# mlysy/rodeo

Hardware: AMD Instinct MI355X
Metric: ODE steps/sec x batch (trajectory-steps/s), FitzHugh-Nagumo q=3, 4000 steps, solve_mv (higher is better)
Workload: dtype f64

## Files before the change

### rodeo_amd/csrc/embed_sources.py

```python
#!/usr/bin/env python3
import os
import sys

HEADERS = ["rk_enums.hpp", "linalg_small.hpp", "kalman_small.hpp", "philox.hpp", "solve_args.hpp", "dual.hpp",
           "sqrt_small.hpp", "solve_small_kernels.hpp", "mfma_tile.hpp", "solve_tile3_kernels.hpp",
           "solve_tile4_kernels.hpp", "solve_tilen_kernels.hpp", "solve_sqrt_kernels.hpp", "solve_small_m_kernels.hpp",
           "solve_dense_itg_kernels.hpp", "dalton_kernels.hpp", "dalton_tile3_kernels.hpp", "rhs.hpp", "dual2.hpp",
           "daltonng_kernels.hpp", "dalton_at_kernels.hpp", "dalton_at_tile3_kernels.hpp", "evidence_kernels.hpp",
           "evidence_tile3_kernels.hpp", "dynamic_kernels.hpp"]
here = os.path.dirname(os.path.abspath(__file__))
out = sys.argv[1]
with open(out, "w") as f:
    f.write("// generated by embed_sources.py -- do not edit\n")
    f.write("static const char* const kJitHeaderNames[] = {%s};\n" % ", ".join('"%s"' % h for h in HEADERS))
    f.write("static const char* const kJitHeaderSources[] = {\n")
    for h in HEADERS:
        src = open(os.path.join(here, h)).read()
        assert ')RKSRC"' not in src
        chunks = [src[i:i + 8000] for i in range(0, len(src), 8000)]
        f.write("    " + "\n    ".join('R"RKSRC(%s)RKSRC"' % c for c in chunks) + ",\n")
    f.write("};\nstatic const int kJitNumHeaders = %d;\n" % len(HEADERS))
```

### rodeo_amd/csrc/solve_args.hpp

```cpp
#pragma once
#ifndef __HIPCC_RTC__
#include <hip/hip_runtime.h>
#endif
#include <stdint.h>

namespace rk {

struct SolveArgs {
    int B, N, D;
    double t_min, t_max;
    uint64_t seed, traj_offset;
    const double *W, *x0, *Q, *R, *theta;
    int W_b, x0_b, Q_b, R_b, theta_b;
    double *mean, *var, *mean_pred, *var_pred, *x;
};

__device__ __forceinline__ double ld(const double* p, size_t e, int batched, int B, int b) {
    return batched ? p[e * (size_t)B + b] : p[e];
}

template <int P>
__device__ __forceinline__ void load_block_consts(const SolveArgs& a, int blk, int b, double (&Q)[P][P],
                                                  double (&R)[P][P]) {
#pragma unroll
    for (int i = 0; i < P; ++i)
#pragma unroll
        for (int j = 0; j < P; ++j) {
            const size_t e = ((size_t)blk * P + i) * P + j;
            Q[i][j] = ld(a.Q, e, a.Q_b, a.B, b);
            R[i][j] = ld(a.R, e, a.R_b, a.B, b);
        }
}

}
```

### rodeo_amd/csrc/solve_tile3.hip

```cpp
#include <cstdlib>
#include "common.hpp"
#include "kalman_small.hpp"
#include "mfma_tile.hpp"
#include "philox.hpp"
#include "rhs.hpp"
#include "solve_args.hpp"
#include "solve_paths.hpp"
#include "solve_tile3_kernels.hpp"
#include "fenrir_at_args.hpp"

namespace rk {

constexpr int CHUNK = 16;
constexpr int ITEM_BYTES = 3 * 128;
constexpr int BUF_BYTES = CHUNK * 4 * ITEM_BYTES;
constexpr int ZONE_BYTES = 64 * TILE_DOUBLES * 8;

__device__ __forceinline__ int lds_byte(int s, int g, int which, int idx) {
    const int item = s * 4 + g;
    return item * ITEM_BYTES + which * 128 + (tile_slot(s, g, idx) << 3);
}

__device__ __forceinline__ void tile3_gain_producers(const SolveArgs& a, const double* __restrict__ tiles, int D, int tw, int wave,
                                                     int lane, int n_tiles, size_t tstride, int n_chunks, char* lds_raw,
                                                     char* zones) {
    constexpr int P = 3;
    const int p = wave - 1;
    const int s = lane >> 2, g = lane & 3;
    int tau = tw * 4 + g;
    if (tau >= n_tiles) tau = n_tiles - 1;
    const int b = tau / D, blk = tau - b * D;
    double Q[P][P], R[P][P];
    load_block_consts<P>(a, blk, b, Q, R);
    int woff[12];
#pragma unroll
    for (int i = 0; i < 3; ++i)
#pragma unroll
        for (int j = 0; j < 4; ++j) woff[i * 4 + j] = lds_byte(s, g, 0, i * 4 + j);
    char* const zone = zones + p * ZONE_BYTES;
    const unsigned zone_lds = __builtin_amdgcn_readfirstlane(lds_addr(zone));
    int frow[6], fcol[6];
#pragma unroll
    for (int i = 0; i < 6; ++i) { const int j = 64 * i + lane; frow[i] = j / 24; fcol[i] = (j % 24) * 16; }
    const char* const wave_tiles = (const char*)(tiles + (size_t)tw * 4 * TILE_DOUBLES);
    auto fetch = [&](int ch) {
        const int n_hi = a.N - 1 - ch * CHUNK;
#pragma unroll
        for (int i = 0; i < 6; ++i) {
            const int n = n_hi - frow[i];
            lds_dma16(wave_tiles + (size_t)(n < 1 ? 1 : n) * tstride * 8 + fcol[i], zone_lds + 1024 * i);
        }
    };
    lds_dma_wait_all();
    if (p < n_chunks) fetch(p);
    double mf[P], Sf[P][P], mp[P], Sp[P][P], A[P][P], X[P][P], rpiv[P];
    for (int t = -3; t < n_chunks; ++t) {
        const int ch1 = t + 3, ch2 = t + 2, ch3 = t + 1;
        if (ch1 % 3 == p) {
            if (ch1 < n_chunks) {
                lds_dma_wait_all();
                double buf[TILE_DOUBLES];
#pragma unroll
                for (int k = 0; k < 6; ++k) {
                    const double2 v = *(const double2*)(zone + 96 * lane + 16 * k);
                    buf[2 * k] = v.x; buf[2 * k + 1] = v.y;
                }
                lds_reads_done();
                if (ch1 + 3 < n_chunks) fetch(ch1 + 3);
#pragma unroll
                for (int i = 0; i < P; ++i) {
#pragma unroll
                    for (int j = 0; j < P; ++j) Sf[i][j] = buf[i * 4 + j];
                    mf[i] = buf[i * 4 + 3];
                }
                predict_block<P>(Q, R, mf, Sf, mp, Sp);
            }
        } else if (ch2 >= 0 && ch2 % 3 == p) {
            if (ch2 < n_chunks) {
                double T[P][P];
                mm_nt<P, P, P>(Sf, Q, T);
#pragma unroll
                for (int i = 0; i < P; ++i)
#pragma unroll
                    for (int j = 0; j < P; ++j) { A[i][j] = Sp[i][j]; X[i][j] = T[j][i]; }
                lu_factor_fwd<P, P>(A, X, rpiv);
            }
        } else if (ch3 >= 0) {
            if (ch3 < n_chunks) {
                lu_back<P, P>(A, X, rpiv);
                const int n = a.N - 1 - ch3 * CHUNK - s;
                if (n >= 1) {
                    char* o = lds_raw + (ch3 & 1) * BUF_BYTES;
#pragma unroll
                    for (int i = 0; i < P; ++i) {
#pragma unroll
                        for (int j = 0; j < P; ++j) {
                            *(double*)(o + woff[i * 4 + j]) = Sp[i][j];
                            *(double*)(o + woff[i * 4 + j] + 128) = X[i][j];
                            *(double*)(o + woff[i * 4 + j] + 256) = Sf[i][j];
                        }
                        *(double*)(o + woff[i * 4 + 3]) = mp[i];
                        *(double*)(o + woff[i * 4 + 3] + 256) = mf[i];
                    }
                }
            }
        }
        lds_barrier();   
    }
}

__global__ void __launch_bounds__(256) bwd_mv_tile3_kernel(SolveArgs a, double* __restrict__ tiles, int D) {
    __shared__ __attribute__((aligned(16))) char lds_all[2 * BUF_BYTES];
    __shared__ __attribute__((aligned(16))) char zones[3 * ZONE_BYTES];
    const int wave = threadIdx.x >> 6, lane = threadIdx.x & 63;
    const int n_tiles = a.B * D;
    const size_t tstride = (size_t)n_tiles * TILE_DOUBLES;
    const int n_chunks = (a.N - 1 + CHUNK - 1) / CHUNK;

    for (int i = threadIdx.x; i < 2 * 64 * 3 * 16; i += 256) {
        const int idx = i & 15, which = (i >> 4) % 3, item = ((i >> 4) / 3) & 63, buf = i / (64 * 3 * 16);
        const double v = (idx == 15) ? 1.0 : 0.0;
        *(double*)(lds_all + buf * BUF_BYTES + lds_byte(item >> 2, item & 3, which, idx)) = v;
    }
    __syncthreads();

    const int tw = blockIdx.x;
    char* const lds_raw = lds_all;
    double* const dump = tiles + (size_t)(a.N + 1) * tstride + (size_t)tw * 64;
    const int role = wave;

    if (role >= 1) {
        tile3_gain_producers(a, tiles, D, tw, role, lane, n_tiles, tstride, n_chunks, lds_raw, zones);
    } else {
        const TileCoord tc = tile_coord<1>(tw, lane, n_tiles);
        __builtin_amdgcn_s_setprio(3);
        const int r = tc.r, g = tc.g, c = tc.c, idx = r * 4 + c;
        const bool st = tc.valid && r < 3;
        double* base = st ? tiles + (size_t)tc.tau * TILE_DOUBLES + idx : dump + lane;
        const size_t ostride = st ? tstride : 0;
        int roff[4];
#pragma unroll
        for (int k = 0; k < 4; ++k) roff[k] = lds_byte(k, g, 0, idx) - k * 4 * ITEM_BYTES;
        double Ms = st ? base[(size_t)a.N * ostride] : ((r == 3 && c == 3) ? 1.0 : 0.0);
        const char* const wave_rows = (const char*)(tiles + (size_t)tw * 4 * TILE_DOUBLES);
        const size_t row_bytes = tstride * sizeof(double);
        const unsigned bvoff = st ? (unsigned)((g * TILE_DOUBLES + idx) * sizeof(double)) : 0x80000000u;
        const bool buffer_ok = (CHUNK - 1) * row_bytes + 384 < 0x7fffffffull;
        const int chunk_span = (int)((CHUNK - 1) * row_bytes + 384);
        lds_barrier();
        lds_barrier();
        lds_barrier();
        for (int t = 0; t < n_chunks; ++t) {
            const char* in = lds_raw + (t & 1) * BUF_BYTES;
            const int n_hi = a.N - 1 - t * CHUNK;
            const int cnt = __builtin_amdgcn_readfirstlane(n_hi >= CHUNK ? CHUNK : n_hi);
            double* o = base + (size_t)n_hi * ostride;
            {
                if (cnt == CHUNK && buffer_ok) {
                    constexpr int LOOKAHEAD = 4;
                    double Mp[CHUNK], Gt[CHUNK], Mf[CHUNK];
                    auto load = [&](int s) {
                        const char* q = in + roff[s & 3] + s * 4 * ITEM_BYTES;
                        Mp[s] = *(const double*)(q);
                        Gt[s] = *(const double*)(q + 128);
                        Mf[s] = *(const double*)(q + 256);
                    };
#pragma unroll
                    for (int s = 0; s < LOOKAHEAD; ++s) load(s);
                    const __amdgpu_buffer_rsrc_t rsrc = __builtin_amdgcn_make_buffer_rsrc(
                        (void*)(wave_rows + (size_t)(n_hi - (CHUNK - 1)) * row_bytes), 0, chunk_span, 0x00020000);
                    double Dm = Ms - Mp[0];
#pragma unroll
                    for (int s = 0; s < CHUNK; ++s) {
                        if (s + LOOKAHEAD < CHUNK) load(s + LOOKAHEAD);
                        __builtin_amdgcn_sched_barrier(0);
                        const double V1 = MF(Dm, Gt[s], 0.0);
                        Ms = MF(V1, Gt[s], Mf[s]);
                        if (s + 1 < CHUNK) Dm = Ms - Mp[s + 1];
                        u32x2 bits;
                        __builtin_memcpy(&bits, &Ms, 8);
                        __builtin_amdgcn_raw_buffer_store_b64(bits, rsrc, (int)bvoff, (int)((CHUNK - 1 - s) * row_bytes), 0);
                        __builtin_amdgcn_sched_barrier(0);
                    }
                } else {
                    for (int s = 0; s < cnt; ++s) {
                        const char* q = in + lds_byte(s, g, 0, idx);
                        const double Mp = *(const double*)(q), Gt = *(const double*)(q + 128), Mf = *(const double*)(q + 256);
                        const double V1 = MF(Ms - Mp, Gt, 0.0);
                        Ms = MF(V1, Gt, Mf);
                        o[0] = Ms;
                        o -= ostride;
                    }
                }
            }
            lds_barrier();   
        }
    }
}

struct FenrirObs {
    const double *obs, *obs_w, *obs_v;
    const int32_t* obs_ind;
    int n_obs;
    double* logdens;
};

template <bool AT, class OB>
__device__ __forceinline__ void fenrir_tile3_body(const SolveArgs& a, const double* __restrict__ tiles, int D, const OB& ob) {
    __shared__ __attribute__((aligned(16))) char lds_all[2 * BUF_BYTES];
    __shared__ __attribute__((aligned(16))) char zones[3 * ZONE_BYTES];
    const int wave = threadIdx.x >> 6, lane = threadIdx.x & 63;
    const int n_tiles = a.B * D;
    const size_t tstride = (size_t)n_tiles * TILE_DOUBLES;
    const int n_chunks = (a.N - 1 + CHUNK - 1) / CHUNK;

    for (int i = threadIdx.x; i < 2 * 64 * 3 * 16; i += 256) {
        const int idx = i & 15, which = (i >> 4) % 3, item = ((i >> 4) / 3) & 63, buf = i / (64 * 3 * 16);
        const double v = (idx == 15) ? 1.0 : 0.0;
        *(double*)(lds_all + buf * BUF_BYTES + lds_byte(item >> 2, item & 3, which, idx)) = v;
    }
    __syncthreads();

    const int tw = blockIdx.x;
    char* const lds_raw = lds_all;

    if (wave >= 1) {
        tile3_gain_producers(a, tiles, D, tw, wave, lane, n_tiles, tstride, n_chunks, lds_raw, zones);
    } else {
        __builtin_amdgcn_s_setprio(3);
        const int r = lane >> 4, g = (lane >> 2) & 3, c = lane & 3, idx = r * 4 + c;
        const int tau_raw = tw * 4 + g;
        const bool valid = tau_raw < n_tiles;
        const int tau = valid ? tau_raw : n_tiles - 1;
        const int b = tau / D, blk = tau - b * D;
        const bool in_tile = valid && r < 3;
        const double e3 = (r == 3 && c == 3) ? 1.0 : 0.0, I4 = r == c ? 1.0 : 0.0;
        const double* const my = tiles + (size_t)tau * TILE_DOUBLES + idx;
        int roff[4];
#pragma unroll
        for (int k = 0; k < 4; ++k) roff[k] = lds_byte(k, g, 0, idx) - k * 4 * ITEM_BYTES;
        double Ms = in_tile ? my[(size_t)a.N * tstride] : e3;
        double acc = 0.0;
        int i = ob.n_obs - 1;
        int next = -1;
        [[maybe_unused]] int off = 0;
        auto look = [&]() {
            if constexpr (AT) {
                next = i >= 0 ? ob.tab[4 * i] : -1;
                off = i >= 0 ? ob.tab[4 * i + 1] : 0;
            } else {
                next = i >= 0 ? ob.obs_ind[i] : -1;
            }
        };
        look();
        auto observe = [&]() {
            const double xw = valid ? (r < 3 ? ob.obs_w[((size_t)i * D + blk) * 3 + r] : -ob.obs[(size_t)i * D + blk]) : 0.0;
            const double Om = valid ? ob.obs_v[(size_t)i * D + blk] : 1.0;
            double MsT = MF(Ms, I4, 0.0);
            MsT = r == 3 ? 0.0 : MsT;
            const double WS = MF(xw, Ms, 0.0);
            const double Z = MF(MsT, xw, 0.0);
            const double w = MF(Z, xw, 0.0) + Om;
            const double z = -quad_bcast3(WS);
            if (fabs(w) > 1e-8) acc += -0.5 * (z * z / w + log(w)) - 0.5 * 1.83787706640934548356;
            const double K = Z / w;
            Ms = fma(-K, WS, Ms);
            --i;
            look();
        };
        auto step = [&](double Mp, double Gt, double Mf) {
            const double V1 = MF(Ms - Mp, Gt, 0.0);
            Ms = MF(V1, Gt, Mf);
        };
        [[maybe_unused]] auto interval = [&](int n, bool to_node) {
            if constexpr (AT) {
                const double* const my_hops = ob.hops + (size_t)tau * FENRIR_AT_TILE_REC + idx;
                const int n_rec = ob.n_pre + ob.n_post;
                auto hop = [&](int rec) {
                    const double* q = my_hops + (size_t)fenrir_at_clamp(rec, n_rec) * n_tiles * FENRIR_AT_TILE_REC;
                    step(q[0], q[16], q[32]);
                };
                hop(ob.n_pre + fenrir_at_clamp(ob.tab[4 * i + 3], ob.n_post));
                do {
                    const int pre = fenrir_at_clamp(ob.tab[4 * i + 2], ob.n_pre);
                    observe();
                    if (to_node || (off && next == n)) hop(pre);
                } while (off && next == n);
            }
        };
        if (next >= a.N && !off) observe();
        __syncthreads();
        __syncthreads();
        __syncthreads();
        for (int t = 0; t < n_chunks; ++t) {
            const char* in = lds_raw + (t & 1) * BUF_BYTES;
            const int n_hi = a.N - 1 - t * CHUNK;
            const int cnt = __builtin_amdgcn_readfirstlane(n_hi >= CHUNK ? CHUNK : n_hi);
            const bool has_obs = next > n_hi - cnt;
            if (cnt == CHUNK && !has_obs) {
                constexpr int LOOKAHEAD = 4;
                double Mp[CHUNK], Gt[CHUNK], Mf[CHUNK];
                auto load = [&](int s) {
                    const char* q = in + roff[s & 3] + s * 4 * ITEM_BYTES;
                    Mp[s] = *(const double*)(q);
                    Gt[s] = *(const double*)(q + 128);
                    Mf[s] = *(const double*)(q + 256);
                };
#pragma unroll
                for (int s = 0; s < LOOKAHEAD; ++s) load(s);
                double Dm = Ms - Mp[0];
#pragma unroll
                for (int s = 0; s < CHUNK; ++s) {
                    if (s + LOOKAHEAD < CHUNK) load(s + LOOKAHEAD);
                    __builtin_amdgcn_sched_barrier(0);
                    const double V1 = MF(Dm, Gt[s], 0.0);
                    Ms = MF(V1, Gt[s], Mf[s]);
                    if (s + 1 < CHUNK) Dm = Ms - Mp[s + 1];
                    __builtin_amdgcn_sched_barrier(0);
                }
            } else {
                for (int s = 0; s < cnt; ++s) {
                    const int n = n_hi - s;
                    bool hops = false;
                    if constexpr (AT) hops = off && next == n;
                    if (hops) {
                        interval(n, true);
                    } else {
                        const char* q = in + lds_byte(s, g, 0, idx);
                        step(*(const double*)(q), *(const double*)(q + 128), *(const double*)(q + 256));
                    }
                    if (!off && next == n) observe();
                }
            }
            __syncthreads();
        }
        if constexpr (AT)
            if (off && next == 0) interval(0, false);
        if (!off && next == 0) {
            Ms = in_tile ? my[0] : e3;
            observe();
        }
        if (valid && r == 0 && c == 0) atomicAdd(&ob.logdens[b], acc);
    }
}

__global__ void __launch_bounds__(256) fenrir_bwd_tile3_kernel(SolveArgs a, const double* __restrict__ tiles, int D, FenrirObs ob) {
    fenrir_tile3_body<false>(a, tiles, D, ob);
}

__global__ void __launch_bounds__(256) fenrir_bwd_at_tile3_kernel(SolveArgs a, const double* __restrict__ tiles, int D, FenrirAt ob) {
    fenrir_tile3_body<true>(a, tiles, D, ob);
}

constexpr int SIM_ITEM = 256;
constexpr int SIM_BUF = CHUNK * 4 * SIM_ITEM;

__device__ __forceinline__ int sim_tile_byte(int s, int g, int idx) {
    const int item = s * 4 + g;
    return item * SIM_ITEM + (tile_slot(s, g, idx) << 3);
}
__device__ __forceinline__ int sim_vec_byte(int s, int g, int which, int rr) {
    const int item = s * 4 + g;
    return item * SIM_ITEM + 128 + (vec_slot(s, g, which, rr) << 3);
}

struct SimLogpost {
    const double* obs;
    const int32_t* obs_ind;
    int n_obs;
    double noise_sd;
    const double* upars;
    int n_prior;
    double prior_sd;
    double* logpost;
};
constexpr int LP_MAX_OBS = 512, LP_MAX_VALS = 1024;

template <bool LP>
__global__ void __launch_bounds__(256, 2) bwd_sim_tile3_kernel(SolveArgs a, double* __restrict__ tiles, int D, SimLogpost lp) {
    constexpr int P = 3;
    __shared__ double lp_obs[LP ? LP_MAX_VALS : 1];
    __shared__ int lp_ind[LP ? LP_MAX_OBS : 1];
    if constexpr (LP) {
        for (int i = threadIdx.x; i < lp.n_obs * D; i += 256) lp_obs[i] = lp.obs[i];
        for (int i = threadIdx.x; i < lp.n_obs; i += 256) { const int ni = lp.obs_ind[i]; lp_ind[i] = ni < 0 ? 0 : (ni > a.N ? a.N : ni); }
    }
    __shared__ __attribute__((aligned(16))) char lds_all[2 * SIM_BUF];
    __shared__ __attribute__((aligned(16))) char zones[3 * ZONE_BYTES];
    constexpr int QR_STRIDE = 2 * 9 + 2;
    __shared__ __attribute__((aligned(16))) double qr[4 * QR_STRIDE];
    const int wave = threadIdx.x >> 6, lane = threadIdx.x & 63;
    const int n_tiles = a.B * D;
    const size_t tstride = (size_t)n_tiles * TILE_DOUBLES;
    const int n_chunks = (a.N + CHUNK - 1) / CHUNK;
    for (int i = threadIdx.x; i < 2 * SIM_BUF / 8; i += 256) ((double*)lds_all)[i] = 0.0;
    __syncthreads();
    const int tw = blockIdx.x;
    char* const lds_raw = lds_all;
    double* const dump = tiles + (size_t)(a.N + 1) * tstride + (size_t)tw * 64;

    if (wave >= 1) {
        const int p = wave - 1;
        const int s = lane >> 2, g = lane & 3;
        int tau = tw * 4 + g;
        if (tau >= n_tiles) tau = n_tiles - 1;
        const int b = tau / D, blk = tau - b * D;
        const uint32_t traj = (uint32_t)(a.traj_offset + (uint64_t)b);
        if (p == 0 && s == 0) {
            double Q0[P][P], R0[P][P];
            load_block_consts<P>(a, blk, b, Q0, R0);
#pragma unroll
            for (int i = 0; i < P; ++i)
#pragma unroll
                for (int j = 0; j < P; ++j) { qr[g * QR_STRIDE + i * P + j] = Q0[i][j]; qr[g * QR_STRIDE + 9 + i * P + j] = R0[i][j]; }
        }
        lds_barrier();
        const double* const my_qr = qr + g * QR_STRIDE;
        auto load_q = [&](double (&Qv)[P][P]) {
#pragma unroll
            for (int i = 0; i < P; ++i)
#pragma unroll
                for (int j = 0; j < P; ++j) Qv[i][j] = my_qr[i * P + j];
        };
        int woff[9], voff[3], voff1[3];
#pragma unroll
        for (int i = 0; i < 3; ++i) {
#pragma unroll
            for (int j = 0; j < 3; ++j) woff[i * 3 + j] = sim_tile_byte(s, g, i * 4 + j);
            voff[i] = sim_vec_byte(s, g, 0, i);
            voff1[i] = sim_vec_byte(s, g, 1, i);
        }
        char* const zone = zones + p * ZONE_BYTES;
        const unsigned zone_lds = __builtin_amdgcn_readfirstlane(lds_addr(zone));
        int frow[6], fcol[6];
#pragma unroll
        for (int i = 0; i < 6; ++i) { const int j = 64 * i + lane; frow[i] = j / 24; fcol[i] = (j % 24) * 16; }
        const char* const wave_tiles = (const char*)(tiles + (size_t)tw * 4 * TILE_DOUBLES);
        auto fetch = [&](int ch) {
            const int n_hi = a.N - ch * CHUNK;
#pragma unroll
            for (int i = 0; i < 6; ++i) {
                const int n = n_hi - frow[i];
                lds_dma16(wave_tiles + (size_t)(n < 1 ? 1 : n) * tstride * 8 + fcol[i], zone_lds + 1024 * i);
            }
        };
        lds_dma_wait_all();
        if (p < n_chunks) fetch(p);
        double mf[P], Sf[P][P], mp[P], Sp[P][P], T[P][P], A[P][P], X[P][P], rpiv[P], z[P];
        for (int t = -3; t < n_chunks; ++t) {
            const int ch1 = t + 3, ch2 = t + 2, ch3 = t + 1;
            if (ch1 % 3 == p) {
                if (ch1 < n_chunks) {
                    lds_dma_wait_all();
                    double buf[TILE_DOUBLES];
#pragma unroll
                    for (int k = 0; k < 6; ++k) {
                        const double2 v = *(const double2*)(zone + 96 * lane + 16 * k);
                        buf[2 * k] = v.x; buf[2 * k + 1] = v.y;
                    }
                    lds_reads_done();
                    if (ch1 + 3 < n_chunks) fetch(ch1 + 3);
#pragma unroll
                    for (int i = 0; i < P; ++i) {
#pragma unroll
                        for (int j = 0; j < P; ++j) Sf[i][j] = buf[i * 4 + j];
                        mf[i] = buf[i * 4 + 3];
                    }
                    {
                        double Q[P][P], R[P][P];
                        load_q(Q);
#pragma unroll
                        for (int i = 0; i < P; ++i)
#pragma unroll
                            for (int j = 0; j < P; ++j) R[i][j] = my_qr[9 + i * P + j];
                        predict_block<P>(Q, R, mf, Sf, mp, Sp);
                    }
                    const int n = a.N - ch1 * CHUNK - s;
#ifdef RK_T3_ABLATE_SIMZ
                    z[0] = 0.25 + 1e-3 * n; z[1] = -0.5;
#else
                    normal_pair(a.seed, traj, (uint32_t)(n < 1 ? 1 : n), (uint32_t)blk, PURPOSE_SMOOTH, 0u, z[0], z[1]);
#endif
                }
            } else if (ch2 >= 0 && ch2 % 3 == p) {
                if (ch2 < n_chunks) {
                    {
                        double Q[P][P];
                        load_q(Q);
                        mm_nt<P, P, P>(Sf, Q, T);
                    }
#pragma unroll
                    for (int i = 0; i < P; ++i)
#pragma unroll
                        for (int j = 0; j < P; ++j) { A[i][j] = Sp[i][j]; X[i][j] = T[j][i]; }
                    lu_factor_fwd<P, P>(A, X, rpiv);
                    const int n = a.N - ch2 * CHUNK - s;
                    double z3;
#ifdef RK_T3_ABLATE_SIMZ
                    z[2] = 0.125 + 1e-3 * n; z3 = 0.0;
#else
                    normal_pair(a.seed, traj, (uint32_t)(n < 1 ? 1 : n), (uint32_t)blk, PURPOSE_SMOOTH, 1u, z[2], z3);
#endif
                }
            } else if (ch3 >= 0) {
                if (ch3 < n_chunks) {
                    const int n = a.N - ch3 * CHUNK - s;
                    double GT[P][P], Ssim[P][P], L[P][P], G[P][P];
                    lu_back<P, P>(A, X, rpiv);
                    const bool term = n == a.N;
#pragma unroll
                    for (int i = 0; i < P; ++i)
#pragma unroll
                        for (int j = 0; j < P; ++j) G[i][j] = term ? 0.0 : X[j][i];
                    mm_nt<P, P, P>(G, T, GT);
#pragma unroll
                    for (int i = 0; i < P; ++i)
#pragma unroll
                        for (int j = 0; j < P; ++j) Ssim[i][j] = Sf[i][j] - GT[i][j];
#ifdef RK_T3_ABLATE_SIMPSD
#pragma unroll
                    for (int i = 0; i < P; ++i)
#pragma unroll
                        for (int j = 0; j < P; ++j) L[i][j] = Ssim[i][j];
#else
                    psd_factor<P>(Ssim, L);
#endif
                    if (n >= 1) {
                        char* o = lds_raw + (ch3 & 1) * SIM_BUF;
#pragma unroll
                        for (int i = 0; i < P; ++i) {
                            double w = mf[i];
#pragma unroll
                            for (int k = 0; k <= i; ++k) w = fma(L[i][k], z[k], w);
#pragma unroll
                            for (int j = 0; j < P; ++j) *(double*)(o + woff[i * 3 + j]) = G[j][i];
                            *(double*)(o + voff[i]) = term ? 0.0 : mp[i];
                            *(double*)(o + voff1[i]) = w;
                        }
                    }
                }
            }
            lds_barrier();
        }
    } else {
        const TileCoord tc = tile_coord<1>(tw, lane, n_tiles);
        const int r = tc.r, g = tc.g, c = tc.c, idx = r * 4 + c;
        const int b = tc.tau / D, blk = tc.tau - b * D;
        const bool st = tc.valid && r < 3 && c == 0 && a.x != nullptr;
        const size_t xstride = (size_t)D * P * a.B;
        double* bx = st ? a.x + ((size_t)blk * P + r) * a.B + b : dump + lane;
        const double LOG_SQRT_2PI = 0.91893853320467274178;
        const double lsd = LP ? log(lp.noise_sd) : 0.0;
        int io = LP ? lp.n_obs - 1 : -1;
        double acc = 0.0;
        auto next_index = [&]() { return io >= 0 ? __builtin_amdgcn_readfirstlane(lp_ind[io]) : -1; };
        auto observe = [&](double xv) {
            const double zz = (lp_obs[io * D + blk] - xv) / lp.noise_sd;
            acc += -0.5 * zz * zz - lsd - LOG_SQRT_2PI;
            --io;
        };
        const size_t sx = st ? xstride : 0;
        const bool xbuf_ok = (size_t)CHUNK * xstride * sizeof(double) < 0x7fffffffull;
        const int xvo = st && xbuf_ok ? (int)((((size_t)blk * P + r) * a.B + b) * sizeof(double)) : (int)0x80000000;
        int roff[4], rvec[4], rvec1[4];
#pragma unroll
        for (int k = 0; k < 4; ++k) {
            roff[k] = sim_tile_byte(k, g, idx) - k * 4 * SIM_ITEM;
            rvec[k] = sim_vec_byte(k, g, 0, r) - k * 4 * SIM_ITEM;
            rvec1[k] = sim_vec_byte(k, g, 1, r) - k * 4 * SIM_ITEM;
        }
        double x = 0.0;
        lds_barrier();
        int next_n = LP ? next_index() : -1;
        lds_barrier();
        lds_barrier();
        lds_barrier();
        for (int t = 0; t < n_chunks; ++t) {
            const char* in = lds_raw + (t & 1) * SIM_BUF;
            const int n_hi = a.N - t * CHUNK;
            const int cnt = __builtin_amdgcn_readfirstlane(n_hi >= CHUNK ? CHUNK : n_hi);
            double* o = bx + (size_t)n_hi * sx;
            auto step = [&](const char* q, const char* qv, const char* qw) {
                const double Gt = *(const double*)(q), mp = *(const double*)(qv), mfw = *(const double*)(qw);
                x = MF(Gt, x - mp, mfw);
                o[0] = x;
                o -= sx;
            };
            int n_cur = n_hi;
            if (cnt == CHUNK && xbuf_ok) {
                const __amdgpu_buffer_rsrc_t rsrc = __builtin_amdgcn_make_buffer_rsrc(
                    (void*)(a.x + (size_t)(n_hi - (CHUNK - 1)) * xstride), 0, (int)(CHUNK * xstride * sizeof(double)), 0x00020000);
                double xs[LP ? CHUNK : 1];
#pragma unroll
                for (int s = 0; s < CHUNK; ++s) {
                    const double Gt = *(const double*)(in + roff[s & 3] + s * 4 * SIM_ITEM);
                    const double mp = *(const double*)(in + rvec[s & 3] + s * 4 * SIM_ITEM);
                    const double mfw = *(const double*)(in + rvec1[s & 3] + s * 4 * SIM_ITEM);
                    x = MF(Gt, x - mp, mfw);
                    u32x2 bits;
                    __builtin_memcpy(&bits, &x, 8);
                    __builtin_amdgcn_raw_buffer_store_b64(bits, rsrc, xvo, (int)((CHUNK - 1 - s) * xstride * sizeof(double)), 0);
                    if constexpr (LP) xs[s] = x;
                }
                if constexpr (LP) {
                    if (next_n > n_hi - CHUNK) {
#pragma unroll
                        for (int s = 0; s < CHUNK; ++s)
                            while (n_hi - s == next_n) { observe(xs[s]); next_n = next_index(); }
                    }
                }
            } else if (cnt == CHUNK) {
#pragma unroll
                for (int s = 0; s < CHUNK; ++s) {
                    step(in + roff[s & 3] + s * 4 * SIM_ITEM, in + rvec[s & 3] + s * 4 * SIM_ITEM, in + rvec1[s & 3] + s * 4 * SIM_ITEM);
                    if constexpr (LP) {
                        while (n_cur == next_n) { observe(x); next_n = next_index(); }
                    }
                    --n_cur;
                }
            } else {
                for (int s = 0; s < cnt; ++s) {
                    step(in + sim_tile_byte(s, g, idx), in + sim_vec_byte(s, g, 0, r), in + sim_vec_byte(s, g, 1, r));
                    if constexpr (LP) {
                        while (n_cur == next_n) { observe(x); next_n = next_index(); }
                    }
                    --n_cur;
                }
            }
            lds_barrier();
        }
        const double x_init = tiles[(size_t)tc.tau * TILE_DOUBLES + r * 4 + 3];
        if (st) bx[0] = x_init;
        if constexpr (LP) {
            while (next_n == 0) { observe(x_init); next_n = next_index(); }
            if (D >= 2) acc += __shfl_xor(acc, 4, 64);
            if (D >= 4) acc += __shfl_xor(acc, 8, 64);
            if (tc.valid && r == 0 && c == 0 && blk == 0) {
                if (lp.upars) {
                    const double lps = log(lp.prior_sd);
                    for (int k = 0; k < lp.n_prior; ++k) {
                        const double zz = lp.upars[(size_t)k * a.B + b] / lp.prior_sd;
                        acc += -0.5 * zz * zz - lps - LOG_SQRT_2PI;
                    }
                }
                lp.logpost[b] = acc;
            }
        }
    }
}

template <class RHS>
static int launch_fwd_tile(rk_handle h, const rk_solve_cfg* c, const SolveArgs& a, double* tiles) {
    const LaunchGeom g = fwd_tile_geom(a.B, RHS::D);
    launch_placement_primer(h, g.grid, g.block);
    LaunchTimer t(h, "fwd_tile3_kernel");
    const bool ok = dispatch_int<RK_INTERROGATE_RODEO, RK_INTERROGATE_CHKREBTII>(c->interrogate, [&](auto I) {
        hipLaunchKernelGGL((fwd_tile3_kernel<RHS, I>), g.grid, g.block, 0, h->stream, a, tiles);
    });
    RK_REQUIRE(ok, RK_ERR_UNSUPPORTED, "tile path: interrogate id %d not supported", c->interrogate);
    t.stop();
    RK_HIP(hipGetLastError());
    return RK_OK;
}

template <int D>
constexpr bool tile_geom_matches() {
    if constexpr (D == 0) return true;
    else return tiles_per_wave(D) == Tpw<D>::value && tile_waves(D) == TileWaves<D>::value && tile_geom_matches<D - 1>();
}
static_assert(tile_geom_matches<TILE_MAX_BLOCKS>(), "tiles_per_wave / tile_waves differ from Tpw<D> / TileWaves<D>");

bool tile3_supported(const rk_solve_cfg* c, int mode) {
    if (c->flags & (RK_FLAG_STORE_PRED | RK_FLAG_BATCH_MINOR)) return false;
    if (c->kalman_type != RK_KALMAN_STANDARD || c->n_bstate != 3 || c->n_bmeas != 1) return false;
    if (c->interrogate < RK_INTERROGATE_RODEO || c->interrogate > RK_INTERROGATE_CHKREBTII) return false;
    if (is_user_rhs(c->rhs_id)) return user_tile_available(c, JIT_TILE3);
    return builtin_has_n_block(c->rhs_id, c->n_block);
}

bool tile3_sim_logpost_supported(const rk_solve_cfg* c, int n_obs) {
    return tile3_supported(c, RK_MODE_SIM) && (c->n_block == 1 || c->n_block == 2 || c->n_block == 4) && n_obs <= LP_MAX_OBS &&
           n_obs * c->n_block <= LP_MAX_VALS;
}

int tile3_solve_sim_logpost(rk_handle h, const rk_solve_cfg* c, const SolveArgs& a, double* tiles, const double* obs,
                            const int32_t* obs_ind, int n_obs, double noise_sd, const double* upars, int n_prior, double prior_sd,
                            double* logpost) {
    SimLogpost lp;
    lp.obs = obs; lp.obs_ind = obs_ind; lp.n_obs = n_obs; lp.noise_sd = noise_sd; lp.upars = upars; lp.n_prior = n_prior;
    lp.prior_sd = prior_sd; lp.logpost = logpost;
    return tile3_solve(h, c, a, tiles, RK_MODE_SIM, &lp);
}

int tile3_solve(rk_handle h, const rk_solve_cfg* c, const SolveArgs& a, double* tiles, int mode, const SimLogpost* lp) {
    int rc = RK_ERR_UNSUPPORTED;
    if (is_user_rhs(c->rhs_id)) rc = user_forward_tile(h, c, a, tiles, JIT_TILE3);
    else with_builtin_rhs(c->rhs_id, [&](auto rhs) { rc = launch_fwd_tile<decltype(rhs)>(h, c, a, tiles); });
    if (rc || mode == RK_MODE_FILTER) return rc;
    return tile3_backward(h, a, tiles, mode, lp);
}

int tile3_backward(rk_handle h, const SolveArgs& a, double* tiles, int mode, const SimLogpost* lp) {
    if (mode == RK_MODE_SIM) {
        LaunchTimer t(h, "bwd_sim_tile3_kernel");
        if (lp) hipLaunchKernelGGL(bwd_sim_tile3_kernel<true>, dim3(div_up(a.B * a.D, 4)), dim3(256), 0, h->stream, a, tiles, a.D, *lp);
        else hipLaunchKernelGGL(bwd_sim_tile3_kernel<false>, dim3(div_up(a.B * a.D, 4)), dim3(256), 0, h->stream, a, tiles, a.D, SimLogpost{});
        t.stop();
        RK_HIP(hipGetLastError());
        return RK_OK;
    }
    if (a.N < 2) return RK_OK;
    LaunchTimer t(h, "bwd_mv_tile3_kernel");
    hipLaunchKernelGGL(bwd_mv_tile3_kernel, dim3(div_up(a.B * a.D, 4)), dim3(256), 0, h->stream, a, tiles, a.D);
    t.stop();
    RK_HIP(hipGetLastError());
    return RK_OK;
}

int tile3_fenrir_backward(rk_handle h, const SolveArgs& a, const double* tiles, const double* obs, const double* obs_w,
                          const double* obs_v, const int32_t* obs_ind, int n_obs, double* logdens) {
    FenrirObs ob;
    ob.obs = obs; ob.obs_w = obs_w; ob.obs_v = obs_v; ob.obs_ind = obs_ind; ob.n_obs = n_obs; ob.logdens = logdens;
    LaunchTimer t(h, "fenrir_bwd_tile3_kernel");
    hipLaunchKernelGGL(fenrir_bwd_tile3_kernel, dim3(div_up(a.B * a.D, 4)), dim3(256), 0, h->stream, a, tiles, a.D, ob);
    t.stop();
    RK_HIP(hipGetLastError());
    return RK_OK;
}

int tile3_fenrir_backward_at(rk_handle h, const SolveArgs& a, const double* tiles, const FenrirAt& ob) {
    LaunchTimer t(h, "fenrir_bwd_at_tile3_kernel");
    hipLaunchKernelGGL(fenrir_bwd_at_tile3_kernel, dim3(div_up(a.B * a.D, 4)), dim3(256), 0, h->stream, a, tiles, a.D, ob);
    t.stop();
    RK_HIP(hipGetLastError());
    return RK_OK;
}

}
```

### rodeo_amd/csrc/solve_tile3_kernels.hpp

```cpp
#pragma once
#include "rk_enums.hpp"
#include "kalman_small.hpp"
#include "mfma_tile.hpp"
#include "philox.hpp"
#include "solve_args.hpp"

namespace rk {

constexpr int TILE_DOUBLES = 12;
typedef unsigned int u32x2 __attribute__((ext_vector_type(2)));

struct TileCoord {
    int r, g, c;
    int tau;
    int b, blk;
    bool valid;
};

template <int D, int TPW = 4>
__device__ __forceinline__ TileCoord tile_coord(int wave, int lane, int n_tiles) {
    TileCoord t;
    t.r = lane >> 4; t.g = (lane >> 2) & 3; t.c = lane & 3;
    const int tau = wave * TPW + t.g;
    t.valid = t.g < TPW && tau < n_tiles;
    t.tau = t.valid ? tau : (wave * TPW < n_tiles ? wave * TPW : n_tiles - 1);
    t.b = t.tau / D; t.blk = t.tau - t.b * D;
    return t;
}

constexpr int TILE_MAX_BLOCKS = 64;

template <int D>
struct TileWaves {
    static constexpr int value = D <= 4 ? 1 : (D + 3) / 4;
};

__device__ __forceinline__ double sqrt_pos_1step(double x) {
    const double rs = __builtin_amdgcn_rsq(x);
    const double g = x * rs, h = 0.5 * rs;
    const double s = fma(fma(-g, g, x), h, g);
    return x > 0.0 ? s : 0.0;
}

template <class RHS, int ITG>
__global__ void __launch_bounds__(64 * TileWaves<RHS::D>::value) fwd_tile3_kernel(SolveArgs a, double* __restrict__ tiles) {
    constexpr int D = RHS::D, P = 3, NW = TileWaves<D>::value, TPW = NW > 1 ? 4 : Tpw<D>::value;
    static_assert(D >= 1 && D <= TILE_MAX_BLOCKS, "tile path: n_block in 1..64");
    static_assert(RHS::NDEP == 1, "tile path: right-hand sides that depend on X[b][0] only");
    const int n_tiles = a.B * D;
    const int wave_in_wg = threadIdx.x >> 6, lane = threadIdx.x & 63;
    TileCoord tc;
    if constexpr (NW == 1) {
        tc = tile_coord<D, TPW>(blockIdx.x, lane, n_tiles);
    } else {
        tc.r = lane >> 4; tc.g = (lane >> 2) & 3; tc.c = lane & 3;
        const int blk_w = wave_in_wg * 4 + tc.g;
        tc.valid = blk_w < D;
        tc.b = blockIdx.x; tc.blk = tc.valid ? blk_w : D - 1;
        tc.tau = tc.b * D + tc.blk;
    }
    const int r = tc.r, c = tc.c, b = tc.b, blk = tc.blk;
    const bool in3 = r < 3 && c < 3;

    const double Qt = in3 ? ld(a.Q, ((size_t)blk * P + c) * P + r, a.Q_b, a.B, b) : ((r == 3 && c == 3) ? 1.0 : 0.0);
    const double Qt0 = in3 ? Qt : 0.0;
    const double Rt = in3 ? ld(a.R, ((size_t)blk * P + r) * P + c, a.R_b, a.B, b) : 0.0;
    const double RtT = in3 ? ld(a.R, ((size_t)blk * P + c) * P + r, a.R_b, a.B, b) : 0.0;
    const double Wr = r < 3 ? ld(a.W, (size_t)blk * P + r, a.W_b, a.B, b) : 0.0;
    const double Y0 = r < 3 ? ld(a.Q, ((size_t)blk * P + 0) * P + r, a.Q_b, a.B, b) : 0.0;
    const double E0 = r == 0 ? 1.0 : 0.0;
    const double e3r = r == 3 ? 1.0 : 0.0;
    double th[RHS::NTHETA];
#pragma unroll
    for (int k = 0; k < RHS::NTHETA; ++k) th[k] = a.theta ? ld(a.theta, k, a.theta_b, a.B, b) : 0.0;
    double c3 = 0.0, c2 = 0.0, c1 = 0.0, co = 0.0, c0 = Wr;
    if constexpr (rhs_has_tile_form<RHS>::value && D == 2) {
        double tk[6];
        RHS::tile_consts(blk, th, tk);
        const bool jac = ITG == RK_INTERROGATE_KRAMER;
        const double k4 = jac ? tk[4] : 0.0, k5 = jac ? tk[5] : 0.0;
        if (r == 3) { c3 = k5 - tk[1]; c1 = k4 - tk[0]; co = -tk[2]; c0 = -tk[3]; }
        if (r == 0) { c2 = -k5; c0 = Wr - k4; }
    }
    __shared__ double zbuf_all[NW][4 * 16];
    double* const zbuf = zbuf_all[wave_in_wg];
    __shared__ double vx[2][NW > 1 ? TILE_MAX_BLOCKS : 1];
    const uint32_t traj = (uint32_t)(a.traj_offset + (uint64_t)b);

    double M = r < 3 ? (c == 3 ? ld(a.x0, (size_t)blk * P + r, a.x0_b, a.B, b) : 0.0) : (c == 3 ? 1.0 : 0.0);
    const bool st = tc.valid && r < 3;
    const size_t row_bytes = (size_t)n_tiles * TILE_DOUBLES * sizeof(double);
    constexpr uint32_t SLICE = TPW * TILE_DOUBLES * sizeof(double), WIN_MAX = 0x7fffffffu - SLICE;
    const int WIN_ROWS = row_bytes <= WIN_MAX ? (int)(WIN_MAX / (uint32_t)row_bytes) : 1;
    const int wave_u = NW == 1 ? 0 : __builtin_amdgcn_readfirstlane(wave_in_wg);
    const char* const row0 = (const char*)(tiles + (NW == 1 ? (size_t)blockIdx.x * TPW : (size_t)blockIdx.x * D + (size_t)wave_u * 4) * TILE_DOUBLES);
    const int bvoff = st ? (int)((tc.g * TILE_DOUBLES + r * 4 + c) * sizeof(double)) : (int)0x80000000;
    __amdgpu_buffer_rsrc_t rsrc;
    uint32_t soff = 0;
    auto open_window = [&](int n0) {
        const int n1 = a.N - n0 < WIN_ROWS ? a.N : n0 + WIN_ROWS;
        rsrc = __builtin_amdgcn_make_buffer_rsrc((void*)(row0 + (size_t)n0 * row_bytes), 0,
                                                 (int)((uint32_t)(n1 - n0 - 1) * (uint32_t)row_bytes + SLICE), 0x00020000);
        soff = 0;
        return n1;
    };
    auto store_last_row = [&](double v) {
        const __amdgpu_buffer_rsrc_t last = __builtin_amdgcn_make_buffer_rsrc((void*)(row0 + (size_t)a.N * row_bytes), 0, (int)SLICE, 0x00020000);
        u32x2 bits;
        __builtin_memcpy(&bits, &v, 8);
        __builtin_amdgcn_raw_buffer_store_b64(bits, last, bvoff, 0, 0);
    };
#define RK_STORE_BEHIND(M_, mfma_result)                                               \
    do {                                                                               \
        asm("" : "+v"(M_) : "v"(mfma_result));                                         \
        u32x2 bits_;                                                                   \
        __builtin_memcpy(&bits_, &M_, 8);                                              \
        __builtin_amdgcn_raw_buffer_store_b64(bits_, rsrc, bvoff, (int)soff, 0);       \
        soff += (uint32_t)row_bytes;                                                   \
        asm volatile("" : "+v"(mfma_result) : : "memory");                             \
    } while (0)

    if constexpr (rhs_has_tile_form<RHS>::value && D == 2 && ITG != RK_INTERROGATE_CHKREBTII) {
#define RK_AFTER(in, res) asm("" : "+v"(in) : "v"(res))
        auto step = [&]() __attribute__((always_inline)) {
            double U = MF(M, Qt, 0.0);
            RK_STORE_BEHIND(M, U);
            double B0 = MF(Y0, M, 0.0);
            RK_AFTER(U, B0);
            double MpT = MF(Qt0, U, RtT);
            RK_AFTER(B0, MpT);
            const double v_own = quad_bcast3(B0);
            const double v_oth = pair_other_quad_uniform(v_own);
            const double Xw = fma(fma(fma(c3, v_own, c2), v_own, c1), v_own, fma(co, v_oth, c0));
            RK_AFTER(U, Xw);
            double Mp = MF(U, Qt, Rt);
            RK_AFTER(MpT, Mp);
            double Z0 = MF(MpT, Xw, 0.0);
            RK_AFTER(Mp, Z0);
            double WS = MF(Xw, Mp, 0.0);
            RK_AFTER(Z0, WS);
            double S = MF(Z0, Xw, 0.0);
            RK_AFTER(WS, S);
            if constexpr (ITG == RK_INTERROGATE_RODEO) S = S + S;
            const double PW = Z0 * WS;
            RK_AFTER(S, PW);
            const double y0 = __builtin_amdgcn_rcp(S);
            const double e = fma(-S, y0, 1.0);
            const double y = fma(y0, fma(e, e, e), y0);
            M = fma(-PW, y, Mp);
        };
        for (int n0 = 0; n0 < a.N;) {
            const int n1 = open_window(n0);
            const uint32_t soff_quads = (uint32_t)((n1 - n0) & ~3) * (uint32_t)row_bytes;
            while (soff != soff_quads) { step(); step(); step(); step(); }
            for (int i = (n1 - n0) & 3; i > 0; --i) step();
            n0 = n1;
        }
        store_last_row(M);
#undef RK_AFTER
#ifdef RK_PLACEMENT_DEBUG
        if (lane == 0) {
            double* tail = tiles + (size_t)(a.N + 1) * n_tiles * TILE_DOUBLES + (size_t)blockIdx.x * 64;
            tail[0] = (double)__builtin_amdgcn_s_getreg((31 << 11) | 4);
            tail[1] = (double)__builtin_amdgcn_s_getreg((31 << 11) | 20);
        }
#endif
        return;
    }
    if constexpr (rhs_has_tile_form<RHS>::value && D == 2 && ITG == RK_INTERROGATE_CHKREBTII) {
        double tk[6];
        RHS::tile_consts(blk, th, tk);
        const double ac3 = -tk[1], ac1 = -tk[0], aco = -tk[2], ac0 = -tk[3];
        const double e3c = c == 3 ? 1.0 : 0.0;
        for (int n = 0, n1 = 0; n < a.N; ++n) {
            if (n == n1) n1 = open_window(n);
#if defined(RK_T3_ABLATE) && RK_T3_ABLATE >= 1
            const double zn = 0.25;
#else
            if ((n & 15) == 0) {
                double z0, z1;
                normal_pair(a.seed, traj, (uint32_t)(n + r * 4 + c), (uint32_t)blk, PURPOSE_INTERROGATE, 0u, z0, z1);
                zbuf[tc.g * 16 + r * 4 + c] = z0;
            }
            const double zn = zbuf[tc.g * 16 + (n & 15)];
#endif
            double U = MF(M, Qt, 0.0);
            RK_STORE_BEHIND(M, U);
            const double Mp = MF(U, Qt, Rt);
            const double MpT = MF(Qt0, U, RtT);
            const double R0 = MF(E0, Mp, 0.0);
            double Z0 = MF(MpT, Wr, 0.0);
            const double WS0 = MF(Wr, Mp, 0.0);
            asm("" : "+v"(Z0) : "v"(WS0));
            double S = MF(Z0, Wr, 0.0);
            S = S + S;
            const double rS = fast_rcp_cubic(S);
            double r0v = R0;
            asm("" : "+v"(r0v) : "v"(rS));
#if defined(RK_T3_ABLATE) && RK_T3_ABLATE >= 2
            const double v_own = fma(quad_bcast0(r0v), zn, quad_bcast3(r0v));
#else
            const double v_own = fma(sqrt_pos_1step(quad_bcast0(r0v)), zn, quad_bcast3(r0v));
#endif
            const double v_oth = pair_other_quad_uniform(v_own);
            const double am = fma(fma(fma(ac3, v_own, 0.0), v_own, ac1), v_own, fma(aco, v_oth, ac0));
            const double WS = fma(e3c, am, WS0);
            const double PW = Z0 * WS;
            M = fma(-PW, rS, Mp);
        }
        store_last_row(M);
        return;
    }
    double l0 = 0.0, l1 = 0.0, l2 = 0.0, l3 = 0.0, l4 = 0.0, XwL = 0.0;
    if constexpr (rhs_has_tile3_form<RHS>::value && D == 3 && NW == 1) {
        double kk[5];
        RHS::tile3_consts(blk, th, kk);
        const bool jac = ITG == RK_INTERROGATE_KRAMER;
        l0 = jac ? 0.0 : -kk[0]; l1 = -kk[1]; l2 = -kk[2]; l3 = -kk[3]; l4 = -kk[4];
        XwL = fma(jac ? -kk[0] : 0.0, E0, Wr);
    }
    for (int n = 0, n1 = 0; n < a.N; ++n) {
        if (n == n1) n1 = open_window(n);
        double U = MF(M, Qt, 0.0);
        RK_STORE_BEHIND(M, U);
        double v_own;
        if constexpr (ITG != RK_INTERROGATE_CHKREBTII) v_own = quad_bcast3(MF(Y0, M, 0.0));
        const double Mp = MF(U, Qt, Rt);
        const double MpT = MF(Qt0, U, RtT);
        if constexpr (ITG == RK_INTERROGATE_CHKREBTII) {
            if ((n & 15) == 0) {
                double z0, z1;
                normal_pair(a.seed, traj, (uint32_t)(n + r * 4 + c), (uint32_t)blk, PURPOSE_INTERROGATE, 0u, z0, z1);
                zbuf[tc.g * 16 + r * 4 + c] = z0;
            }
            const double zn = zbuf[tc.g * 16 + (n & 15)];
            const double R0 = MF(E0, Mp, 0.0);
            const double s00 = quad_bcast0(R0);
            v_own = fma(sqrt(s00 > 0.0 ? s00 : 0.0), zn, quad_bcast3(R0));
        }
        const double t = a.t_min + (a.t_max - a.t_min) * (double)(n + 1) / (double)a.N;
        double Xw;
        if constexpr (rhs_has_tile_form<RHS>::value && D == 2) {
            const double v_oth = pair_other_quad_uniform(v_own);
            Xw = fma(fma(fma(c3, v_own, c2), v_own, c1), v_own, fma(co, v_oth, c0));
        } else if constexpr (rhs_has_tile3_form<RHS>::value && D == 3 && NW == 1) {
            const double n1 = from_next_tile(v_own), p1 = from_prev_tile(v_own), p2 = dpp64<0x128>(v_own);
            const double a_meas = fma(l4, p2 * p1, fma(l3, p1 * n1, fma(l2, p1, fma(l1, n1, l0 * v_own))));
            Xw = fma(a_meas, e3r, XwL);
        } else {
            constexpr int PX = 1;
            double X[D][PX];
            if constexpr (NW == 1) {
                double vals[D];
                gather_blocks<D>(v_own, vals);
#pragma unroll
                for (int bb = 0; bb < D; ++bb) X[bb][0] = vals[bb];
            } else {
                if (tc.valid && r == 0 && c == 0) vx[n & 1][blk] = v_own;
                __syncthreads();
#pragma unroll
                for (int bb = 0; bb < D; ++bb) X[bb][0] = vx[n & 1][bb];
            }
            double fb, J0;
            if constexpr (ITG == RK_INTERROGATE_KRAMER && rhs_has_fjac0<RHS>::value) {
                RHS::template fjac0_block<PX>(X, t, th, blk, fb, J0);
            } else if constexpr (ITG != RK_INTERROGATE_KRAMER && rhs_has_f_block<RHS>::value) {
                fb = RHS::template f_block<PX>(X, t, th, blk);
                J0 = 0.0;
            } else {
                double f[D], J[D][PX];
                if constexpr (ITG == RK_INTERROGATE_KRAMER) {
                    RHS::template fjac<PX>(X, t, th, f, J);
                } else {
                    RHS::template f<PX>(X, t, th, f);
#pragma unroll
                    for (int bb = 0; bb < D; ++bb)
#pragma unroll
                        for (int j = 0; j < PX; ++j) J[bb][j] = 0.0;
                }
                double J0s[D];
#pragma unroll
                for (int bb = 0; bb < D; ++bb) J0s[bb] = J[bb][0];
                fb = pick_block<D>(f, blk); J0 = pick_block<D>(J0s, blk);
            }
            const double a_meas = fma(J0, v_own, -fb);
            Xw = fma(-J0, E0, fma(a_meas, e3r, Wr));
        }
        const double WS = MF(Xw, Mp, 0.0);
        const double Z0 = MF(MpT, Xw, 0.0);
        double S = MF(Z0, Xw, 0.0);
        if constexpr (ITG == RK_INTERROGATE_RODEO || ITG == RK_INTERROGATE_CHKREBTII)
            S = S + S;
        const double K = Z0 * fast_rcp_cubic(S);
        M = fma(-K, WS, Mp);
    }
    store_last_row(M);
#undef RK_STORE_BEHIND
}

}
```

Measured before the change: 5.990 billion.

## Pack symmetric filter tiles to cut forward-pass store and producer fetch traffic

In mean-variance mode the forward tile kernel now writes only the upper triangle of each 3x3 covariance plus the mean, 9 doubles instead of 12. Four steps are packed into three stripes of rows. The gain-producer waves fetch this compact layout into LDS and rebuild the symmetric matrices. This lowers global store and reload bandwidth for the per-step filter history. The cost is more complex address arithmetic, a separate path for partial waves, and a dependency on the step count and array size limits.

```diff
diff --git a/rodeo_amd/csrc/embed_sources.py b/rodeo_amd/csrc/embed_sources.py
--- a/rodeo_amd/csrc/embed_sources.py
+++ b/rodeo_amd/csrc/embed_sources.py
@@ -3,7 +3,7 @@
 import sys
 
 HEADERS = ["rk_enums.hpp", "linalg_small.hpp", "kalman_small.hpp", "philox.hpp", "solve_args.hpp", "dual.hpp",
-           "sqrt_small.hpp", "solve_small_kernels.hpp", "mfma_tile.hpp", "solve_tile3_kernels.hpp",
+           "sqrt_small.hpp", "solve_small_kernels.hpp", "mfma_tile.hpp", "tile3_pack.hpp", "solve_tile3_kernels.hpp",
            "solve_tile4_kernels.hpp", "solve_tilen_kernels.hpp", "solve_sqrt_kernels.hpp", "solve_small_m_kernels.hpp",
            "solve_dense_itg_kernels.hpp", "dalton_kernels.hpp", "dalton_tile3_kernels.hpp", "rhs.hpp", "dual2.hpp",
            "daltonng_kernels.hpp", "dalton_at_kernels.hpp", "dalton_at_tile3_kernels.hpp", "evidence_kernels.hpp",
diff --git a/rodeo_amd/csrc/solve_args.hpp b/rodeo_amd/csrc/solve_args.hpp
--- a/rodeo_amd/csrc/solve_args.hpp
+++ b/rodeo_amd/csrc/solve_args.hpp
@@ -12,6 +12,7 @@
     uint64_t seed, traj_offset;
     const double *W, *x0, *Q, *R, *theta;
     int W_b, x0_b, Q_b, R_b, theta_b;
+    int pack = 0;
     double *mean, *var, *mean_pred, *var_pred, *x;
 };
 
diff --git a/rodeo_amd/csrc/solve_tile3.hip b/rodeo_amd/csrc/solve_tile3.hip
--- a/rodeo_amd/csrc/solve_tile3.hip
+++ b/rodeo_amd/csrc/solve_tile3.hip
@@ -21,9 +21,11 @@
     return item * ITEM_BYTES + which * 128 + (tile_slot(s, g, idx) << 3);
 }
 
+enum { FILT_NATURAL = 0, FILT_NATURAL_SYM = 1, FILT_PACKED = 2 };
+
 __device__ __forceinline__ void tile3_gain_producers(const SolveArgs& a, const double* __restrict__ tiles, int D, int tw, int wave,
                                                      int lane, int n_tiles, size_t tstride, int n_chunks, char* lds_raw,
-                                                     char* zones) {
+                                                     char* zones, const int filt) {
     constexpr int P = 3;
     const int p = wave - 1;
     const int s = lane >> 2, g = lane & 3;
@@ -43,8 +45,18 @@
 #pragma unroll
     for (int i = 0; i < 6; ++i) { const int j = 64 * i + lane; frow[i] = j / 24; fcol[i] = (j % 24) * 16; }
     const char* const wave_tiles = (const char*)(tiles + (size_t)tw * 4 * TILE_DOUBLES);
+    auto chunk_lo = [&](int ch) { const int n_lo = a.N - CHUNK - ch * CHUNK; return n_lo < 1 ? 1 : n_lo; };
     auto fetch = [&](int ch) {
         const int n_hi = a.N - 1 - ch * CHUNK;
+        if (filt == FILT_PACKED) {
+            const int n_lo = chunk_lo(ch), n_rows = tile3_pack_chunk_rows(n_lo, n_hi);
+            const char* const first = wave_tiles + (size_t)tile3_pack_chunk_first_row(n_lo) * tstride * 8;
+#pragma unroll
+            for (int i = 0; i < 6; ++i) {
+                if (frow[i] < n_rows) lds_dma16(first + (size_t)frow[i] * tstride * 8 + fcol[i], zone_lds + 1024 * i);
+            }
+            return;
+        }
 #pragma unroll
         for (int i = 0; i < 6; ++i) {
             const int n = n_hi - frow[i];
@@ -60,17 +72,28 @@
             if (ch1 < n_chunks) {
                 lds_dma_wait_all();
                 double buf[TILE_DOUBLES];
-#pragma unroll
-                for (int k = 0; k < 6; ++k) {
-                    const double2 v = *(const double2*)(zone + 96 * lane + 16 * k);
-                    buf[2 * k] = v.x; buf[2 * k + 1] = v.y;
+                if (filt == FILT_PACKED) {
+                    const int n_lo = chunk_lo(ch1), n = a.N - 1 - ch1 * CHUNK - s;
+                    const double* const rec = (const double*)(zone + tile3_pack_zone_byte(n_lo, n < n_lo ? n_lo : n, g));
+#pragma unroll
+                    for (int i = 0; i < P; ++i) {
+#pragma unroll
+                        for (int j = i; j < P; ++j) buf[i * 4 + j] = buf[j * 4 + i] = rec[tile3_pack_slot(i, j)];
+                        buf[i * 4 + 3] = rec[tile3_pack_slot(i, 3)];
+                    }
+                } else {
+#pragma unroll
+                    for (int k = 0; k < 6; ++k) {
+                        const double2 v = *(const double2*)(zone + 96 * lane + 16 * k);
+                        buf[2 * k] = v.x; buf[2 * k + 1] = v.y;
+                    }
                 }
                 lds_reads_done();
                 if (ch1 + 3 < n_chunks) fetch(ch1 + 3);
 #pragma unroll
                 for (int i = 0; i < P; ++i) {
 #pragma unroll
-                    for (int j = 0; j < P; ++j) Sf[i][j] = buf[i * 4 + j];
+                    for (int j = 0; j < P; ++j) Sf[i][j] = buf[filt == FILT_NATURAL || i <= j ? i * 4 + j : j * 4 + i];
                     mf[i] = buf[i * 4 + 3];
                 }
                 predict_block<P>(Q, R, mf, Sf, mp, Sp);
@@ -130,7 +153,10 @@
     const int role = wave;
 
     if (role >= 1) {
-        tile3_gain_producers(a, tiles, D, tw, role, lane, n_tiles, tstride, n_chunks, lds_raw, zones);
+        if (a.pack && tile3_pack_full_wave(tw, n_tiles))
+            tile3_gain_producers(a, tiles, D, tw, role, lane, n_tiles, tstride, n_chunks, lds_raw, zones, FILT_PACKED);
+        else
+            tile3_gain_producers(a, tiles, D, tw, role, lane, n_tiles, tstride, n_chunks, lds_raw, zones, FILT_NATURAL_SYM);
     } else {
         const TileCoord tc = tile_coord<1>(tw, lane, n_tiles);
         __builtin_amdgcn_s_setprio(3);
@@ -193,7 +219,7 @@
                     }
                 }
             }
-            lds_barrier();   
+            lds_barrier();
         }
     }
 }
@@ -225,7 +251,7 @@
     char* const lds_raw = lds_all;
 
     if (wave >= 1) {
-        tile3_gain_producers(a, tiles, D, tw, wave, lane, n_tiles, tstride, n_chunks, lds_raw, zones);
+        tile3_gain_producers(a, tiles, D, tw, wave, lane, n_tiles, tstride, n_chunks, lds_raw, zones, FILT_NATURAL);
     } else {
         __builtin_amdgcn_s_setprio(3);
         const int r = lane >> 4, g = (lane >> 2) & 3, c = lane & 3, idx = r * 4 + c;
@@ -692,12 +718,25 @@
     return tile3_solve(h, c, a, tiles, RK_MODE_SIM, &lp);
 }
 
+template <class RHS>
+static bool tile3_packs(const rk_solve_cfg* c, const SolveArgs& a, int mode) {
+    if (!(rhs_has_tile_form<RHS>::value && RHS::D == 2) || mode != RK_MODE_MV || c->interrogate == RK_INTERROGATE_CHKREBTII) return false;
+    const char* const force = getenv("RK_TILE3_PACK");
+    if (force && force[0] == '0') return false;
+    const size_t array_bytes = (size_t)(a.N + 1) * a.B * RHS::D * TILE_DOUBLES * sizeof(double);
+    return a.N >= T3P_MIN_STEPS && array_bytes < 0x7fff0000ull;
+}
+
 int tile3_solve(rk_handle h, const rk_solve_cfg* c, const SolveArgs& a, double* tiles, int mode, const SimLogpost* lp) {
     int rc = RK_ERR_UNSUPPORTED;
+    SolveArgs ap = a;
     if (is_user_rhs(c->rhs_id)) rc = user_forward_tile(h, c, a, tiles, JIT_TILE3);
-    else with_builtin_rhs(c->rhs_id, [&](auto rhs) { rc = launch_fwd_tile<decltype(rhs)>(h, c, a, tiles); });
+    else with_builtin_rhs(c->rhs_id, [&](auto rhs) {
+        ap.pack = tile3_packs<decltype(rhs)>(c, a, mode);
+        rc = launch_fwd_tile<decltype(rhs)>(h, c, ap, tiles);
+    });
     if (rc || mode == RK_MODE_FILTER) return rc;
-    return tile3_backward(h, a, tiles, mode, lp);
+    return tile3_backward(h, ap, tiles, mode, lp);
 }
 
 int tile3_backward(rk_handle h, const SolveArgs& a, double* tiles, int mode, const SimLogpost* lp) {
diff --git a/rodeo_amd/csrc/solve_tile3_kernels.hpp b/rodeo_amd/csrc/solve_tile3_kernels.hpp
--- a/rodeo_amd/csrc/solve_tile3_kernels.hpp
+++ b/rodeo_amd/csrc/solve_tile3_kernels.hpp
@@ -4,6 +4,7 @@
 #include "mfma_tile.hpp"
 #include "philox.hpp"
 #include "solve_args.hpp"
+#include "tile3_pack.hpp"
 
 namespace rk {
 
@@ -110,21 +111,38 @@
         __builtin_memcpy(&bits, &v, 8);
         __builtin_amdgcn_raw_buffer_store_b64(bits, last, bvoff, 0, 0);
     };
-#define RK_STORE_BEHIND(M_, mfma_result)                                               \
+#define RK_STORE_AT(M_, mfma_result, voff_, adv_)                                      \
     do {                                                                               \
         asm("" : "+v"(M_) : "v"(mfma_result));                                         \
         u32x2 bits_;                                                                   \
         __builtin_memcpy(&bits_, &M_, 8);                                              \
-        __builtin_amdgcn_raw_buffer_store_b64(bits_, rsrc, bvoff, (int)soff, 0);       \
-        soff += (uint32_t)row_bytes;                                                   \
+        __builtin_amdgcn_raw_buffer_store_b64(bits_, rsrc, voff_, (int)soff, 0);       \
+        soff += (adv_);                                                                \
         asm volatile("" : "+v"(mfma_result) : : "memory");                             \
     } while (0)
+#define RK_STORE_BEHIND(M_, mfma_result) RK_STORE_AT(M_, mfma_result, bvoff, (uint32_t)row_bytes)
 
     if constexpr (rhs_has_tile_form<RHS>::value && D == 2 && ITG != RK_INTERROGATE_CHKREBTII) {
 #define RK_AFTER(in, res) asm("" : "+v"(in) : "v"(res))
-        auto step = [&]() __attribute__((always_inline)) {
+        const bool pack = a.pack && tile3_pack_full_wave(blockIdx.x, n_tiles);
+        int voff[4];
+#pragma unroll
+        for (int j = 0; j < 4; ++j) {
+            const int gb = tile3_pack_group_byte(j, tc.g, tile3_pack_slot(r < 3 ? r : 0, c));
+            const uint32_t packed = (uint32_t)tile3_pack_row(0, gb) * (uint32_t)row_bytes + (uint32_t)tile3_pack_col(gb);
+            const bool slot = st && (!pack || tile3_pack_slot(r, c) >= 0);
+            voff[j] = slot ? (int)(pack ? packed : (uint32_t)bvoff + (uint32_t)j * (uint32_t)row_bytes) : (int)0x80000000;
+        }
+        const uint32_t quad_bytes = (pack ? 3u : 4u) * (uint32_t)row_bytes;
+        if (pack) {
+            const __amdgpu_buffer_rsrc_t first = __builtin_amdgcn_make_buffer_rsrc((void*)row0, 0, (int)SLICE, 0x00020000);
+            u32x2 bits;
+            __builtin_memcpy(&bits, &M, 8);
+            __builtin_amdgcn_raw_buffer_store_b64(bits, first, bvoff, 0, 0);
+        }
+        auto step = [&](int vo) __attribute__((always_inline)) {
             double U = MF(M, Qt, 0.0);
-            RK_STORE_BEHIND(M, U);
+            RK_STORE_AT(M, U, vo, 0u);
             double B0 = MF(Y0, M, 0.0);
             RK_AFTER(U, B0);
             double MpT = MF(Qt0, U, RtT);
@@ -151,9 +169,12 @@
         };
         for (int n0 = 0; n0 < a.N;) {
             const int n1 = open_window(n0);
-            const uint32_t soff_quads = (uint32_t)((n1 - n0) & ~3) * (uint32_t)row_bytes;
-            while (soff != soff_quads) { step(); step(); step(); step(); }
-            for (int i = (n1 - n0) & 3; i > 0; --i) step();
+            const uint32_t soff_quads = (uint32_t)((n1 - n0) >> 2) * quad_bytes;
+            while (soff != soff_quads) { step(voff[0]); step(voff[1]); step(voff[2]); step(voff[3]); soff += quad_bytes; }
+            const int tail = (n1 - n0) & 3;
+            if (tail > 0) step(voff[0]);
+            if (tail > 1) step(voff[1]);
+            if (tail > 2) step(voff[2]);
             n0 = n1;
         }
         store_last_row(M);
@@ -296,6 +317,7 @@
     }
     store_last_row(M);
 #undef RK_STORE_BEHIND
+#undef RK_STORE_AT
 }
 
 }
diff --git a/rodeo_amd/csrc/tile3_pack.hpp b/rodeo_amd/csrc/tile3_pack.hpp
--- /dev/null
+++ b/rodeo_amd/csrc/tile3_pack.hpp
@@ -0,0 +1,27 @@
+#pragma once
+
+namespace rk {
+
+constexpr int T3P_STRIPE = 384;
+constexpr int T3P_REC = 72;
+constexpr int T3P_STEP = 4 * T3P_REC;
+constexpr int T3P_GROUP = 4 * T3P_STEP;
+constexpr int T3P_MIN_STEPS = 16;
+static_assert(T3P_GROUP == 3 * T3P_STRIPE, "four packed steps are three stripes");
+
+constexpr bool tile3_pack_full_wave(int tw, int n_tiles) { return 4 * tw + 4 <= n_tiles; }
+
+constexpr int tile3_pack_slot(int r, int c) {
+    return c == 3 ? 6 + r : (c < r ? -1 : (r == 0 ? c : (r == 1 ? 2 + c : 5)));
+}
+constexpr int tile3_pack_group_byte(int n, int g, int slot) { return (n & 3) * T3P_STEP + g * T3P_REC + slot * 8; }
+constexpr int tile3_pack_row(int k, int gb) { return 3 * k + 1 + gb / T3P_STRIPE; }
+constexpr int tile3_pack_col(int gb) { return gb % T3P_STRIPE; }
+
+constexpr int tile3_pack_chunk_first_row(int n_lo) { return 3 * (n_lo >> 2) + 1; }
+constexpr int tile3_pack_chunk_rows(int n_lo, int n_hi) { return 3 * ((n_hi >> 2) - (n_lo >> 2) + 1); }
+constexpr int tile3_pack_zone_byte(int n_lo, int n, int g) {
+    return ((n >> 2) - (n_lo >> 2)) * T3P_GROUP + (n & 3) * T3P_STEP + g * T3P_REC;
+}
+
+}
```

After: 6.194 billion, median of 6. 1.03x the previous value.
